# kei312/stereoanywhere

Measured on AMD Instinct MI355X. Metric: stereo pairs/sec @540x960 D=192 (1/2/4/8 GPU) + EPE vs reference, higher is better.
Workload: dtype f32 (F(4x4) Winograd-domain and direct-conv products as exact f16 hi/lo pair products on MFMA, fp32 accumulation; everything else fp32); 1 GPU; configs[1]: batch 4/GPU x 540x960 (padded 544x960), 22 GRU iters, published flags; global_batch=4, iters=22, parallelism=dp1 (independent pairs, metrics all_gather)

## Files before the change

### stereoanywhere_amd/csrc/conv_direct.hip

```cpp
#include "sa_common.h"

#pragma clang fp contract(fast)

namespace {

using sa::f32x4, sa::f32x2, sa::f16x2, sa::f16x4;

constexpr float DSP_SCALE = 4096.0f;
__device__ __forceinline__ f16x4 dsplit(const float x) {
  const f16x2 hh = __builtin_convertvector(f32x2{x, x}, f16x2);
  float l;
  asm("v_fma_mix_f32 %0, -%1, 1.0, %2 op_sel_hi:[1,0,0]" : "=v"(l) : "v"(__builtin_bit_cast(unsigned, hh)), "v"(x));
  const f16x2 ll = __builtin_convertvector(f32x2{l, l}, f16x2);
  return __builtin_shufflevector(hh, ll, 0, 1, 2, 3);
}

__device__ __forceinline__ float dunsplit(const float packed) {
  const f16x2 p = __builtin_bit_cast(f16x2, packed);
  return (float)p[0] + (float)p[1];
}

__device__ unsigned g_direct_redo_blocks;

constexpr int DOTH = 8, DOTW = 32, MT = 2;

template <int K, int S, int KC, int NTL, bool DS>
struct DCfg {
  static constexpr int PH = (DOTH - 1) * S + K, PW = (DOTW - 1) * S + K;
  static constexpr int PWP = PW;
  static constexpr int PL0 = PH * PWP, PR = S == 1 ? 16 : 17;
  static constexpr int PLANE = PL0 + ((PR - PL0 % 32) + 32) % 32;
  static constexpr int XN = KC * PLANE;
  static constexpr int NC = 16 * NTL;
  static constexpr int KK = K * K;
  static constexpr int WN = KC * KK * NC;
  static constexpr int DN = DS ? KC * NC : 0;
  static constexpr int NCP = NC + 16;
  static constexpr int WROWS = KC * KK + (DS ? KC : 0);
  static constexpr int XPT = (XN + 511) / 512, WPT = (WN + DN) / 4 / 512 + (((WN + DN) / 4) % 512 ? 1 : 0);
  static constexpr int KSTEPS = KC * KK / 4;
  static constexpr int NACC = NTL * (DS ? 2 : 1);
  static constexpr int SMEM = XN + WROWS * NCP + 4;
  static_assert(KC % 4 == 0, "a K-step of 4 must stay inside one tap");
  static_assert((WN + DN) % 4 == 0, "weights are staged as float4");
  static_assert(SMEM * 4 <= 160 * 1024, "LDS budget");
  static_assert(8 * 2 * NACC * 16 * 2 <= SMEM, "the stats reduction reuses the staging LDS");
};

struct DirArgs {
  const float *in;
  long in_bs;
  const float *skip, *cm, *cs;
  long skip_bs;
  int Cin, H, W, Ho, Wo;
  const float *wg, *wd;
  int Cout, co_blocks, tiles_w, tiles, nchunks;
  float *out, *out_ds;
  long out_bs, out_ds_bs;
  double *part, *part_ds;
};

__device__ __forceinline__ float close_value(float v, float m, float s, float k) {
#pragma clang fp contract(off)
  const float y = fmaxf((v - m) * s + 0.0f, 0.0f);
  return fmaxf(y + k, 0.0f);
}

template <int K, int S, int KC, int NTL, bool DS, bool SP = false, bool CL = false>
__global__ __launch_bounds__(512, DS ? 2 : 4) void conv_direct_kernel(const DirArgs a) {
  using C = DCfg<K, S, KC, NTL, DS>;
  constexpr int NC = C::NC, NCP = C::NCP, PLANE = C::PLANE, PWP = C::PWP;
  __shared__ __attribute__((aligned(16))) float sm[C::SMEM];
  __shared__ float ctab[CL ? 2 : 1][CL ? 2 * KC : 1];
  float *sx = sm, *sw = sm + C::XN, *sd = sw + KC * C::KK * NCP;
  constexpr int SPARE = C::SMEM - 4;
  const int tid = threadIdx.x, lane = tid & 63;
  const int wv = __builtin_amdgcn_readfirstlane(tid >> 6);
  const unsigned wid = sa::xcd_remap(blockIdx.x, gridDim.x);
  const int cb = wid % a.co_blocks;
  const int st = (wid / a.co_blocks) % a.tiles;
  const int n = wid / (a.co_blocks * a.tiles);
  const int oy0 = (st / a.tiles_w) * DOTH, ox0 = (st % a.tiles_w) * DOTW;
  const int iy0 = oy0 * S - K / 2, ix0 = ox0 * S - K / 2;
  const long hw = (long)a.H * a.W;
  const float *src = a.in + (long)n * a.in_bs;

  constexpr int OOB = 0x7ffffff0;
  const __amdgpu_buffer_rsrc_t xin = __builtin_amdgcn_make_buffer_rsrc(
      const_cast<float *>(src), (short)0, (int)((long)a.Cin * hw * 4), 0x00020000);
  int xoff[C::XPT], xl[C::XPT];
#pragma unroll
  for (int j = 0; j < C::XPT; ++j) {
    const int i = tid + 512 * j;
    const int ci = i / PLANE, rem = i % PLANE, r = rem / PWP, c = rem % PWP;
    const int y = iy0 + r, x = ix0 + c;
    const bool ok = i < C::XN && rem < C::PH * PWP && c < C::PW && y >= 0 && y < a.H && x >= 0 && x < a.W;
    xoff[j] = ok ? (int)((min(ci, a.Cin - 1) * hw + (long)y * a.W + x) * 4) : OOB;
    xl[j] = i < C::XN ? i : SPARE;
  }
  constexpr int WQ = (C::WN + C::DN) / 4;
  const __amdgpu_buffer_rsrc_t win = __builtin_amdgcn_make_buffer_rsrc(
      const_cast<float *>(a.wg) + (long)cb * a.nchunks * C::WN, (short)0, (int)((long)a.nchunks * C::WN * 4),
      0x00020000);
  const __amdgpu_buffer_rsrc_t din = __builtin_amdgcn_make_buffer_rsrc(
      const_cast<float *>(DS ? a.wd + (long)cb * a.nchunks * C::DN : a.wg), (short)0,
      (int)((long)a.nchunks * (DS ? C::DN : 0) * 4), 0x00020000);
  int woff[C::WPT], wl[C::WPT];
  bool wds[C::WPT];
#pragma unroll
  for (int j = 0; j < C::WPT; ++j) {
    const int i = tid + 512 * j;
    wds[j] = i >= C::WN / 4;
    woff[j] = i < WQ ? (wds[j] ? (i - C::WN / 4) * 16 : i * 16) : OOB;
    const int row = (4 * i) / NC, col = (4 * i) % NC;
    wl[j] = i < WQ ? row * NCP + col : SPARE;
  }
  const __amdgpu_buffer_rsrc_t kin = __builtin_amdgcn_make_buffer_rsrc(
      const_cast<float *>(CL ? a.skip + (long)n * a.skip_bs : src), (short)0, (int)((long)a.Cin * hw * 4), 0x00020000);
  float xr[C::XPT], kr[CL ? C::XPT : 1];
  float tv = 0.0f;
  f32x4 wr[C::WPT];
  auto fetch = [&](int chunk) __attribute__((always_inline)) {
    const int xs = chunk * KC * (int)hw * 4;
#pragma unroll
    for (int j = 0; j < C::XPT; ++j) xr[j] = __uint_as_float(__builtin_amdgcn_raw_buffer_load_b32(xin, xoff[j], xs, 0));
    if constexpr (CL) {
#pragma unroll
      for (int j = 0; j < C::XPT; ++j) kr[j] = __uint_as_float(__builtin_amdgcn_raw_buffer_load_b32(kin, xoff[j], xs, 0));
      if (tid < 2 * KC) {
        const int c = min(chunk * KC + tid % KC, a.Cin - 1);
        tv = (tid < KC ? a.cm : a.cs)[(long)n * a.Cin + c];
      }
    }
#pragma unroll
    for (int j = 0; j < C::WPT; ++j) {
      const auto v = wds[j] ? __builtin_amdgcn_raw_buffer_load_b128(din, woff[j], chunk * C::DN * 4, 0)
                            : __builtin_amdgcn_raw_buffer_load_b128(win, woff[j], chunk * C::WN * 4, 0);
      wr[j] = f32x4{__uint_as_float(v[0]), __uint_as_float(v[1]), __uint_as_float(v[2]), __uint_as_float(v[3])};
    }
  };
  auto put_tab = [&](int chunk) __attribute__((always_inline)) {
    if (CL && tid < 2 * KC) ctab[CL ? chunk & 1 : 0][tid] = tv;
  };
  auto commit = [&](int chunk) __attribute__((always_inline)) {
#pragma unroll
    for (int j = 0; j < C::XPT; ++j) {
      float v = xr[j];
      if constexpr (CL) {
        const int cl = min((tid + 512 * j) / PLANE, KC - 1);
        const float *tb = ctab[chunk & 1];
        v = xoff[j] == OOB ? 0.0f : close_value(v, tb[cl], tb[KC + cl], kr[j]);
      }
      sx[xl[j]] = v;
    }
#pragma unroll
    for (int j = 0; j < C::WPT; ++j) *reinterpret_cast<f32x4 *>(sw + wl[j]) = wr[j];
  };

  f32x4 acc[MT][C::NACC];
#pragma unroll
  for (int m = 0; m < MT; ++m)
#pragma unroll
    for (int t = 0; t < C::NACC; ++t) acc[m][t] = f32x4{0.f, 0.f, 0.f, 0.f};
  const int kq = lane >> 4, ml = lane & 15;
  int abase[MT];
#pragma unroll
  for (int m = 0; m < MT; ++m) abase[m] = kq * PLANE + (wv * S) * PWP + (m * 16 + ml) * S;
  const int bbase = kq * NCP + ml;

  fetch(0);
  if constexpr (CL) {
    put_tab(0);
    __syncthreads();
  }
  commit(0);
  __syncthreads();
#pragma unroll 1
  for (int chunk = 0; chunk < a.nchunks; ++chunk) {
    if (chunk + 1 < a.nchunks) fetch(chunk + 1);
#pragma unroll
    for (int s = 0; s < C::KSTEPS; ++s) {
      const int tap = (4 * s) / KC, ci0 = (4 * s) % KC;
      const int koff = ci0 * PLANE + (tap / K) * PWP + (tap % K);
      float av[MT];
#pragma unroll
      for (int m = 0; m < MT; ++m) av[m] = sx[abase[m] + koff];
      auto prod = [&](const float bv, f32x4 *ac) __attribute__((always_inline)) {
        if constexpr (SP) {
          const f16x4 b = __builtin_bit_cast(f16x4, f32x2{bv, bv});
#pragma unroll
          for (int m = 0; m < MT; ++m) ac[m * C::NACC] = __builtin_amdgcn_mfma_f32_16x16x16f16(dsplit(av[m]), b, ac[m * C::NACC], 0, 0, 0);
        } else {
#pragma unroll
          for (int m = 0; m < MT; ++m) ac[m * C::NACC] = __builtin_amdgcn_mfma_f32_16x16x4f32(av[m], bv, ac[m * C::NACC], 0, 0, 0);
        }
      };
#pragma unroll
      for (int t = 0; t < NTL; ++t) prod(sw[bbase + 4 * s * NCP + t * 16], &acc[0][t]);
      if (DS && tap == (K / 2) * K + K / 2) {
#pragma unroll
        for (int t = 0; t < NTL; ++t) prod(sd[bbase + ci0 * NCP + t * 16], &acc[0][NTL + t]);
      }
    }
    if (CL && chunk + 1 < a.nchunks) put_tab(chunk + 1);
    __syncthreads();
    if (chunk + 1 < a.nchunks) {
      commit(chunk + 1);
      __syncthreads();
    }
  }
  if constexpr (SP) {
    f32x4 sum = f32x4{0.f, 0.f, 0.f, 0.f};
#pragma unroll
    for (int m = 0; m < MT; ++m)
#pragma unroll
      for (int t = 0; t < C::NACC; ++t) sum += acc[m][t];
    const float tot = (sum.x + sum.y) + (sum.z + sum.w);
    if (__syncthreads_or(!__builtin_isfinite(tot))) {
      if (tid == 0) atomicAdd(&g_direct_redo_blocks, 1u);
#pragma unroll
      for (int m = 0; m < MT; ++m)
#pragma unroll
        for (int t = 0; t < C::NACC; ++t) acc[m][t] = f32x4{0.f, 0.f, 0.f, 0.f};
#pragma unroll 1
      for (int chunk = 0; chunk < a.nchunks; ++chunk) {
        fetch(chunk);
        if constexpr (CL) {
          put_tab(chunk);
          __syncthreads();
        }
        commit(chunk);
        __syncthreads();
#pragma unroll 1
        for (int s = 0; s < C::KSTEPS; ++s) {
          const int tap = (4 * s) / KC, ci0 = (4 * s) % KC;
          const int koff = ci0 * PLANE + (tap / K) * PWP + (tap % K);
#pragma unroll
          for (int t = 0; t < NTL; ++t) {
            const float w = dunsplit(sw[bbase + 4 * s * NCP + t * 16]);
#pragma unroll
            for (int m = 0; m < MT; ++m)
              acc[m][t] = __builtin_amdgcn_mfma_f32_16x16x4f32(sx[abase[m] + koff], w, acc[m][t], 0, 0, 0);
          }
          if (DS && tap == (K / 2) * K + K / 2) {
#pragma unroll
            for (int t = 0; t < NTL; ++t) {
              const float w = dunsplit(sd[bbase + ci0 * NCP + t * 16]);
#pragma unroll
              for (int m = 0; m < MT; ++m)
                acc[m][NTL + t] = __builtin_amdgcn_mfma_f32_16x16x4f32(sx[abase[m] + koff], w, acc[m][NTL + t], 0, 0, 0);
            }
          }
        }
        __syncthreads();
      }
    }
  }

  if constexpr (SP) {
#pragma unroll
    for (int m = 0; m < MT; ++m)
#pragma unroll
      for (int t = 0; t < C::NACC; ++t) acc[m][t] *= 1.0f / DSP_SCALE;
  }
  double *red = reinterpret_cast<double *>(sm);
  constexpr int RC = C::NACC * 16;
  const int oy = oy0 + wv;
  const bool stats = a.part != nullptr;
  const bool interior = oy0 + DOTH <= a.Ho && ox0 + DOTW <= a.Wo && (a.Wo & 3) == 0;
#pragma unroll
  for (int t = 0; t < C::NACC; ++t) {
    const bool ds = DS && t >= NTL;
    const int co = cb * NC + (ds ? t - NTL : t) * 16 + ml;
    float *dst = (ds ? a.out_ds + (long)n * a.out_ds_bs : a.out + (long)n * a.out_bs) + (long)co * a.Ho * a.Wo;
    double s1 = 0.0, s2 = 0.0;
    if (interior) {
#pragma unroll
      for (int m = 0; m < MT; ++m) {
        const int ox = ox0 + m * 16 + 4 * kq;
        *reinterpret_cast<float4 *>(dst + (long)oy * a.Wo + ox) =
            make_float4(acc[m][t][0], acc[m][t][1], acc[m][t][2], acc[m][t][3]);
#pragma unroll
        for (int r = 0; r < 4; ++r) {
          const double v = acc[m][t][r];
          s1 += v;
          s2 += v * v;
        }
      }
    } else {
#pragma unroll
      for (int m = 0; m < MT; ++m) {
        const int ox = ox0 + m * 16 + 4 * kq;
#pragma unroll
        for (int r = 0; r < 4; ++r) {
          if (oy < a.Ho && ox + r < a.Wo) {
            const float v = acc[m][t][r];
            dst[(long)oy * a.Wo + ox + r] = v;
            s1 += (double)v;
            s2 += (double)v * v;
          }
        }
      }
    }
    if (stats) {
      s1 += __shfl_xor(s1, 16);
      s2 += __shfl_xor(s2, 16);
      s1 += __shfl_xor(s1, 32);
      s2 += __shfl_xor(s2, 32);
      if (kq == 0) {
        red[(wv * 2 + 0) * RC + t * 16 + ml] = s1;
        red[(wv * 2 + 1) * RC + t * 16 + ml] = s2;
      }
    }
  }
  if (stats) {
    __syncthreads();
    for (int c = tid; c < RC; c += 512) {
      double s1 = 0.0, s2 = 0.0;
#pragma unroll
      for (int w = 0; w < 8; ++w) {
        s1 += red[(w * 2 + 0) * RC + c];
        s2 += red[(w * 2 + 1) * RC + c];
      }
      const bool ds = DS && c >= NC;
      double *pp = ds ? a.part_ds : a.part;
      if (pp) {
        const int co = cb * NC + (ds ? c - NC : c);
        pp += (((long)n * a.Cout + co) * a.tiles + st) * 2;
        pp[0] = s1;
        pp[1] = s2;
      }
    }
  }
}

__global__ void direct_weights_kernel(const float *__restrict__ w, int Cout, int Cin, int K, int KC, int NC,
                                      int nchunks, int ds, float *__restrict__ out) {
  const long total = (long)Cout * nchunks * KC * K * K;
  const long i = (long)blockIdx.x * blockDim.x + threadIdx.x;
  if (i >= total) return;
  const int n = (int)(i % NC);
  long r = i / NC;
  const int ci = (int)(r % KC);
  r /= KC;
  const int tap = (int)(r % (K * K));
  r /= K * K;
  const int chunk = (int)(r % nchunks);
  const int cblk = (int)(r / nchunks);
  const int co = cblk * NC + n, cin = chunk * KC + ci;
  (void)ds;
  out[i] = cin < Cin ? w[((long)co * Cin + cin) * K * K + tap] : 0.0f;
}

bool pick(int K, int S, int Cout, int &KC, int &NTL) {
  KC = K == 7 ? 4 : 8;
  if (K == 7 && S == 1 && Cout % 64 == 0) { NTL = 4; return true; }
  if ((K == 3 || K == 1) && S == 2 && Cout == 96) { NTL = 6; return true; }
  if ((K == 3 || K == 1) && S == 2 && Cout % 128 == 0) { NTL = 8; return true; }
  return false;
}

}

extern "C" int sa_conv_direct_weights(const float *weight, int Cout, int Cin, int K, int S, int with_ds,
                                      float *out, void *stream) {
  int KC = 0, NTL = 0;
  SA_REQUIRE(weight && out && Cout > 0 && Cin > 0, "sa_conv_direct_weights: bad arguments");
  SA_REQUIRE(pick(K, S, Cout, KC, NTL) && (K != 1 || with_ds), "sa_conv_direct_weights: no kernel for K=%d S=%d Cout=%d",
             K, S, Cout);
  const int NC = 16 * NTL, nchunks = (Cin + KC - 1) / KC;
  const long total = (long)Cout * nchunks * KC * K * K;
  hipStream_t s = sa::as_stream(stream);
  direct_weights_kernel<<<(unsigned)((total + 255) / 256), 256, 0, s>>>(weight, Cout, Cin, K, KC, NC, nchunks, 0,
                                                                       out);
  return sa::check_launch("sa_conv_direct_weights");
}

namespace {
__global__ void direct_split_kernel(const float *__restrict__ w, long n, unsigned *__restrict__ out) {
  const long i = (long)blockIdx.x * blockDim.x + threadIdx.x;
  if (i >= n) return;
  const double u = (double)w[i] * DSP_SCALE;
  const _Float16 hi = (_Float16)(float)u;
  const _Float16 lo = (_Float16)(float)(u - (double)hi);
  out[i] = (unsigned)__builtin_bit_cast(unsigned short, hi) | ((unsigned)__builtin_bit_cast(unsigned short, lo) << 16);
}

}

extern "C" int sa_conv_direct_weights_split(const float *arranged, long n, void *out, void *stream) {
  SA_REQUIRE(arranged && out && n > 0, "sa_conv_direct_weights_split: bad arguments");
  hipStream_t s = sa::as_stream(stream);
  direct_split_kernel<<<(unsigned)((n + 255) / 256), 256, 0, s>>>(arranged, n, static_cast<unsigned *>(out));
  return sa::check_launch("sa_conv_direct_weights_split");
}

long sa_direct_redo_blocks_internal(int reset) {
  return sa::read_redo_counter(g_direct_redo_blocks, reset, false);
}

extern "C" long sa_conv_direct_weights_size(int Cout, int Cin, int K, int S, int with_ds) {
  int KC = 0, NTL = 0;
  if (!pick(K, S, Cout, KC, NTL) || (K == 1 && !with_ds)) return -1;
  return (long)Cout * ((Cin + KC - 1) / KC) * KC * K * K;
}

extern "C" long sa_conv_direct_stat_parts(int Ho, int Wo) {
  return (long)((Wo + DOTW - 1) / DOTW) * ((Ho + DOTH - 1) / DOTH);
}

template <bool SP>
static int conv_direct_launch(const float *in, long in_bs, int N, int Cin, int H, int W, int K, int S,
                              const float *wg, const float *wd, int Cout, float *out, long out_bs, float *out_ds,
                              long out_ds_bs, double *part, double *part_ds, void *stream,
                              const float *skip = nullptr, long skip_bs = 0, const float *cm = nullptr,
                              const float *cs = nullptr) {
  int KC = 0, NTL = 0;
  const bool ds = wd != nullptr, cl = skip != nullptr;
  SA_REQUIRE(in && wg && out && N > 0 && Cin > 0 && H > 0 && W > 0, "sa_conv_direct: bad arguments");
  SA_REQUIRE(!ds || out_ds, "sa_conv_direct: downsample weights without an output");
  SA_REQUIRE(K != 1 && pick(K, S, Cout, KC, NTL) && ds == (S == 2),
             "sa_conv_direct: no kernel for K=%d S=%d Cout=%d ds=%d", K, S, Cout, (int)ds);
  SA_REQUIRE((long)Cin * H * W < (1L << 31), "sa_conv_direct: image too large");
  SA_REQUIRE(Cin % KC == 0 || Cin <= KC, "sa_conv_direct: Cin must be a multiple of %d (or at most %d)", KC, KC);
  SA_REQUIRE(!cl || (cm && cs && K == 3 && Cin % KC == 0),
             "sa_conv_direct_close: needs mean / rstd, a 3x3 stride-2 conv and Cin %% %d == 0", KC);
  const int p = K / 2;
  const int Ho = (H + 2 * p - K) / S + 1, Wo = (W + 2 * p - K) / S + 1;
  const int tiles_w = (Wo + DOTW - 1) / DOTW, tiles = tiles_w * ((Ho + DOTH - 1) / DOTH);
  const int co_blocks = Cout / (16 * NTL);
  const DirArgs a{in, in_bs, skip, cm, cs, skip_bs, Cin, H, W, Ho, Wo, wg, wd, Cout, co_blocks, tiles_w, tiles,
                  (Cin + KC - 1) / KC, out, out_ds, out_bs, out_ds_bs, part, part_ds};
  const long nblk = (long)N * tiles * co_blocks;
  SA_REQUIRE(nblk < (1L << 31), "sa_conv_direct: grid too large");
  hipStream_t s = sa::as_stream(stream);
  sa::TimingScope ts(SA_K_CONV_DIRECT, s);
  if (K == 7) {
    conv_direct_kernel<7, 1, 4, 4, false, SP><<<(unsigned)nblk, 512, 0, s>>>(a);
  } else if (NTL == 6) {
    if (cl) conv_direct_kernel<3, 2, 8, 6, true, SP, true><<<(unsigned)nblk, 512, 0, s>>>(a);
    else conv_direct_kernel<3, 2, 8, 6, true, SP><<<(unsigned)nblk, 512, 0, s>>>(a);
  } else {
    SA_REQUIRE(!cl, "sa_conv_direct_close: no close form for Cout = %d", Cout);
    conv_direct_kernel<3, 2, 8, 8, true, SP><<<(unsigned)nblk, 512, 0, s>>>(a);
  }
  return sa::check_launch("sa_conv_direct");
}

extern "C" int sa_conv_direct(const float *in, long in_bs, int N, int Cin, int H, int W, int K, int S,
                              const float *wg, const float *wd, int Cout, float *out, long out_bs, float *out_ds,
                              long out_ds_bs, double *part, double *part_ds, void *stream) {
  return conv_direct_launch<false>(in, in_bs, N, Cin, H, W, K, S, wg, wd, Cout, out, out_bs, out_ds, out_ds_bs, part,
                                   part_ds, stream);
}

extern "C" int sa_conv_direct_split(const float *in, long in_bs, int N, int Cin, int H, int W, int K, int S,
                                    const void *wg, const void *wd, int Cout, float *out, long out_bs, float *out_ds,
                                    long out_ds_bs, double *part, double *part_ds, void *stream) {
  return conv_direct_launch<true>(in, in_bs, N, Cin, H, W, K, S, static_cast<const float *>(wg),
                                  static_cast<const float *>(wd), Cout, out, out_bs, out_ds, out_ds_bs, part, part_ds,
                                  stream);
}

extern "C" int sa_conv_direct_close_supported(int K, int S, int Cout) {
  int KC = 0, NTL = 0;
  return K == 3 && S == 2 && pick(K, S, Cout, KC, NTL) && NTL == 6 ? 1 : 0;
}

extern "C" int sa_conv_direct_close(const float *c2, long c2_bs, const float *skip, long skip_bs, const float *mean,
                                    const float *rstd, int N, int Cin, int H, int W, int K, int S, const void *wg,
                                    const void *wd, int split, int Cout, float *out, long out_bs, float *out_ds,
                                    long out_ds_bs, double *part, double *part_ds, void *stream) {
  SA_REQUIRE(skip, "sa_conv_direct_close: null skip");
  if (split)
    return conv_direct_launch<true>(c2, c2_bs, N, Cin, H, W, K, S, static_cast<const float *>(wg),
                                    static_cast<const float *>(wd), Cout, out, out_bs, out_ds, out_ds_bs, part, part_ds,
                                    stream, skip, skip_bs, mean, rstd);
  return conv_direct_launch<false>(c2, c2_bs, N, Cin, H, W, K, S, static_cast<const float *>(wg),
                                   static_cast<const float *>(wd), Cout, out, out_bs, out_ds, out_ds_bs, part, part_ds,
                                   stream, skip, skip_bs, mean, rstd);
}
```

Measured before the change: 71.48 pairs/s.

## Add K=32 f16 hi/lo MFMA direct-conv kernel for split-precision path

Adds a new direct-convolution kernel for the split-precision (SP) path. It stages input patches and weights in LDS as separate f16 hi/lo planes, then computes each tap row with three 16x16x32 f16 MFMAs (hi*hi, hi*lo, lo*hi), replacing per-element 16x16x16 MFMAs that split operands at runtime. This cuts the MFMA instruction count and the in-loop conversion work. In exchange it adds more complex LDS layout and staging code, and a redo path with a new range check (overflow or small-magnitude inputs) that falls back to fp32 MFMA. The epilogue is factored into a shared helper.

New measurement: 71.82 pairs/s (median of 6 runs). No clear change (+0.5%).

```diff
diff --git a/stereoanywhere_amd/csrc/conv_direct.hip b/stereoanywhere_amd/csrc/conv_direct.hip
--- a/stereoanywhere_amd/csrc/conv_direct.hip
+++ b/stereoanywhere_amd/csrc/conv_direct.hip
@@ -7,18 +7,6 @@
 using sa::f32x4, sa::f32x2, sa::f16x2, sa::f16x4;
 
 constexpr float DSP_SCALE = 4096.0f;
-__device__ __forceinline__ f16x4 dsplit(const float x) {
-  const f16x2 hh = __builtin_convertvector(f32x2{x, x}, f16x2);
-  float l;
-  asm("v_fma_mix_f32 %0, -%1, 1.0, %2 op_sel_hi:[1,0,0]" : "=v"(l) : "v"(__builtin_bit_cast(unsigned, hh)), "v"(x));
-  const f16x2 ll = __builtin_convertvector(f32x2{l, l}, f16x2);
-  return __builtin_shufflevector(hh, ll, 0, 1, 2, 3);
-}
-
-__device__ __forceinline__ float dunsplit(const float packed) {
-  const f16x2 p = __builtin_bit_cast(f16x2, packed);
-  return (float)p[0] + (float)p[1];
-}
 
 __device__ unsigned g_direct_redo_blocks;
 
@@ -66,7 +54,83 @@
   return fmaxf(y + k, 0.0f);
 }
 
-template <int K, int S, int KC, int NTL, bool DS, bool SP = false, bool CL = false>
+template <int NTL, bool DS>
+__device__ __forceinline__ void direct_epilogue(const DirArgs &a, f32x4 (&acc)[MT][NTL * (DS ? 2 : 1)], double *red,
+                                                const int tid, const int wv, const int n, const int cb, const int st,
+                                                const int oy0, const int ox0) {
+  constexpr int NC = 16 * NTL, NACC = NTL * (DS ? 2 : 1);
+  const int lane = tid & 63, kq = lane >> 4, ml = lane & 15;
+  constexpr int RC = NACC * 16;
+  const int oy = oy0 + wv;
+  const bool stats = a.part != nullptr;
+  const bool interior = oy0 + DOTH <= a.Ho && ox0 + DOTW <= a.Wo && (a.Wo & 3) == 0;
+#pragma unroll
+  for (int t = 0; t < NACC; ++t) {
+    const bool ds = DS && t >= NTL;
+    const int co = cb * NC + (ds ? t - NTL : t) * 16 + ml;
+    float *dst = (ds ? a.out_ds + (long)n * a.out_ds_bs : a.out + (long)n * a.out_bs) + (long)co * a.Ho * a.Wo;
+    double s1 = 0.0, s2 = 0.0;
+    if (interior) {
+#pragma unroll
+      for (int m = 0; m < MT; ++m) {
+        const int ox = ox0 + m * 16 + 4 * kq;
+        *reinterpret_cast<float4 *>(dst + (long)oy * a.Wo + ox) =
+            make_float4(acc[m][t][0], acc[m][t][1], acc[m][t][2], acc[m][t][3]);
+#pragma unroll
+        for (int r = 0; r < 4; ++r) {
+          const double v = acc[m][t][r];
+          s1 += v;
+          s2 += v * v;
+        }
+      }
+    } else {
+#pragma unroll
+      for (int m = 0; m < MT; ++m) {
+        const int ox = ox0 + m * 16 + 4 * kq;
+#pragma unroll
+        for (int r = 0; r < 4; ++r) {
+          if (oy < a.Ho && ox + r < a.Wo) {
+            const float v = acc[m][t][r];
+            dst[(long)oy * a.Wo + ox + r] = v;
+            s1 += (double)v;
+            s2 += (double)v * v;
+          }
+        }
+      }
+    }
+    if (stats) {
+      s1 += __shfl_xor(s1, 16);
+      s2 += __shfl_xor(s2, 16);
+      s1 += __shfl_xor(s1, 32);
+      s2 += __shfl_xor(s2, 32);
+      if (kq == 0) {
+        red[(wv * 2 + 0) * RC + t * 16 + ml] = s1;
+        red[(wv * 2 + 1) * RC + t * 16 + ml] = s2;
+      }
+    }
+  }
+  if (stats) {
+    __syncthreads();
+    for (int c = tid; c < RC; c += 512) {
+      double s1 = 0.0, s2 = 0.0;
+#pragma unroll
+      for (int w = 0; w < 8; ++w) {
+        s1 += red[(w * 2 + 0) * RC + c];
+        s2 += red[(w * 2 + 1) * RC + c];
+      }
+      const bool ds = DS && c >= NC;
+      double *pp = ds ? a.part_ds : a.part;
+      if (pp) {
+        const int co = cb * NC + (ds ? c - NC : c);
+        pp += (((long)n * a.Cout + co) * a.tiles + st) * 2;
+        pp[0] = s1;
+        pp[1] = s2;
+      }
+    }
+  }
+}
+
+template <int K, int S, int KC, int NTL, bool DS, bool CL = false>
 __global__ __launch_bounds__(512, DS ? 2 : 4) void conv_direct_kernel(const DirArgs a) {
   using C = DCfg<K, S, KC, NTL, DS>;
   constexpr int NC = C::NC, NCP = C::NCP, PLANE = C::PLANE, PWP = C::PWP;
@@ -186,14 +250,8 @@
 #pragma unroll
       for (int m = 0; m < MT; ++m) av[m] = sx[abase[m] + koff];
       auto prod = [&](const float bv, f32x4 *ac) __attribute__((always_inline)) {
-        if constexpr (SP) {
-          const f16x4 b = __builtin_bit_cast(f16x4, f32x2{bv, bv});
-#pragma unroll
-          for (int m = 0; m < MT; ++m) ac[m * C::NACC] = __builtin_amdgcn_mfma_f32_16x16x16f16(dsplit(av[m]), b, ac[m * C::NACC], 0, 0, 0);
-        } else {
-#pragma unroll
-          for (int m = 0; m < MT; ++m) ac[m * C::NACC] = __builtin_amdgcn_mfma_f32_16x16x4f32(av[m], bv, ac[m * C::NACC], 0, 0, 0);
-        }
+#pragma unroll
+        for (int m = 0; m < MT; ++m) ac[m * C::NACC] = __builtin_amdgcn_mfma_f32_16x16x4f32(av[m], bv, ac[m * C::NACC], 0, 0, 0);
       };
 #pragma unroll
       for (int t = 0; t < NTL; ++t) prod(sw[bbase + 4 * s * NCP + t * 16], &acc[0][t]);
@@ -209,129 +267,305 @@
       __syncthreads();
     }
   }
-  if constexpr (SP) {
-    f32x4 sum = f32x4{0.f, 0.f, 0.f, 0.f};
+  direct_epilogue<NTL, DS>(a, acc, reinterpret_cast<double *>(sm), tid, wv, n, cb, st, oy0, ox0);
+}
+
+template <int K, int S, int NTL, bool DS>
+struct K32Cfg {
+  static constexpr int KC = K == 7 ? 4 : 8;
+  static constexpr int TPG = 8 / KC;
+  static constexpr int TC = 4 * TPG;
+  static constexpr int GR = (K + TPG - 1) / TPG;
+  static constexpr int PH = (DOTH - 1) * S + K, PWR = (DOTW - 1) * S + K, PW = (DOTW - 1) * S + TC;
+  static constexpr int SLOTB = 2 * KC;
+  static constexpr int IMGB = PW * SLOTB, ROWB = 2 * IMGB;
+  static constexpr int X0 = (IMGB + 16 + 15) / 16 * 16;
+  static constexpr int XB = PH * ROWB, W0 = X0 + XB;
+  static constexpr int RH = 8 / KC, RPT = PH / RH;
+  static constexpr int CX = PW > 64 ? PW - 64 : 0, EXTRA = KC * PH * CX, EPT = EXTRA ? 1 : 0;
+  static_assert(RPT * RH == PH && EXTRA <= 512, "every patch value has one staging slot");
+  static constexpr int NC = 16 * NTL, NACC = NTL * (DS ? 2 : 1);
+  static constexpr int WN = KC * K * K * NC, DN = DS ? KC * NC : 0;
+  static constexpr int WROWS = 4 * (K + (DS ? 1 : 0));
+  static constexpr int WIMG = WROWS * NC * 16;
+  static constexpr int UNITS = K * GR * NC + (DS ? NC : 0), WPT = (UNITS + 511) / 512;
+  static constexpr int SMEMB = W0 + 2 * WIMG;
+  static_assert(TC >= K && (S == 1 || PW % 2 == 0), "a tap row fits one step");
+  static_assert(XB % 16 == 0 && SMEMB <= 160 * 1024, "LDS budget");
+  static_assert(8 * 2 * NACC * 16 * 8 <= SMEMB, "the stats reduction reuses the staging LDS");
+};
+
+using sa::f16x8;
+using u32x4 = __attribute__((ext_vector_type(4))) unsigned;
+
+template <int K, int S, int NTL, bool DS, bool CL = false>
+__global__ __launch_bounds__(512, DS ? 2 : 4) void conv_direct_k32_kernel(const DirArgs a) {
+  using C = K32Cfg<K, S, NTL, DS>;
+  constexpr int KC = C::KC, NC = C::NC, PW = C::PW, ROWB = C::ROWB, IMGB = C::IMGB, SLOTB = C::SLOTB;
+  constexpr int X0 = C::X0, W0 = C::W0, WIMG = C::WIMG;
+  __shared__ __attribute__((aligned(16))) unsigned char smb[C::SMEMB];
+  __shared__ float ctab[CL ? 2 : 1][CL ? 2 * KC : 1];
+  const int tid = threadIdx.x, lane = tid & 63;
+  const int wv = __builtin_amdgcn_readfirstlane(tid >> 6);
+  const unsigned wid = sa::xcd_remap(blockIdx.x, gridDim.x);
+  const int cb = wid % a.co_blocks;
+  const int st = (wid / a.co_blocks) % a.tiles;
+  const int n = wid / (a.co_blocks * a.tiles);
+  const int oy0 = (st / a.tiles_w) * DOTH, ox0 = (st % a.tiles_w) * DOTW;
+  const int iy0 = oy0 * S - K / 2, ix0 = ox0 * S - K / 2;
+  const long hw = (long)a.H * a.W;
+  const float *src = a.in + (long)n * a.in_bs;
+
+  constexpr int OOB = 0x7ffffff0;
+  const __amdgpu_buffer_rsrc_t xin = __builtin_amdgcn_make_buffer_rsrc(
+      const_cast<float *>(src), (short)0, (int)((long)a.Cin * hw * 4), 0x00020000);
+  auto slot_of = [](const int c) { return S == 2 ? (c & 1) * (PW / 2) + (c >> 1) : c; };
+  const int sci = wv % KC, srow0 = (wv / KC) * C::RPT;
+  const bool cok = lane < C::PWR && ix0 + lane >= 0 && ix0 + lane < a.W;
+  const int xoff = cok ? (int)((min(sci, a.Cin - 1) * hw + ix0 + lane) * 4) : OOB;
+  const int xl = X0 + srow0 * ROWB + slot_of(lane) * SLOTB + sci * 2;
+  auto row_ok = [&](const int k) { return iy0 + srow0 + k >= 0 && iy0 + srow0 + k < a.H; };
+  int eoff = OOB, el = 0, ecl = 0;
+  if constexpr (C::EPT) {
+    const int eci = tid / (C::PH * C::CX), rem = tid % (C::PH * C::CX), r = rem / C::CX, c = 64 + rem % C::CX;
+    const int y = iy0 + r, x = ix0 + c;
+    const bool ok = tid < C::EXTRA && c < C::PWR && y >= 0 && y < a.H && x >= 0 && x < a.W;
+    eoff = ok ? (int)((min(eci, a.Cin - 1) * hw + (long)y * a.W + x) * 4) : OOB;
+    el = tid < C::EXTRA ? X0 + r * ROWB + slot_of(c) * SLOTB + eci * 2 : 0;
+    ecl = min(eci, KC - 1);
+  }
+  const unsigned *wgb = reinterpret_cast<const unsigned *>(a.wg) + (long)cb * a.nchunks * C::WN;
+  const unsigned *wdb = DS ? reinterpret_cast<const unsigned *>(a.wd) + (long)cb * a.nchunks * C::DN : wgb;
+  unsigned wu[C::WPT];
+  static_assert(C::WN + C::DN < 65536 && (W0 + WIMG) / 16 < 65535, "weight units are packed in one register");
+  bool wds[C::WPT], wpad[C::WPT];
+#pragma unroll
+  for (int j = 0; j < C::WPT; ++j) {
+    const int u = tid + 512 * j;
+    const bool valid = u < C::UNITS;
+    wds[j] = DS && valid && u >= K * C::GR * NC;
+    const int v = !valid ? 0 : wds[j] ? u - K * C::GR * NC : u;
+    const int nn = v % NC, sg = v / NC, s = sg / C::GR, g = sg % C::GR;
+    const unsigned wo = wds[j] ? nn : (s * K + g * C::TPG) * KC * NC + nn;
+    wpad[j] = C::TPG == 2 && g * 2 + 1 >= K;
+    wu[j] = wo | (valid ? (unsigned)(W0 / 16 + (wds[j] ? 4 * K + 1 : s * 4 + g) * NC + nn) << 16 : 0xffff0000u);
+  }
+  const __amdgpu_buffer_rsrc_t kin = __builtin_amdgcn_make_buffer_rsrc(
+      const_cast<float *>(CL ? a.skip + (long)n * a.skip_bs : src), (short)0, (int)((long)a.Cin * hw * 4), 0x00020000);
+  constexpr int XPT = C::RPT + C::EPT;
+  float xr[XPT], kr[CL ? XPT : 1];
+  float tv = 0.0f;
+  unsigned wr[C::WPT][8];
+  auto fetch_x = [&](int chunk) __attribute__((always_inline)) {
+    const int xs = chunk * KC * (int)hw * 4;
+#pragma unroll
+    for (int k = 0; k < C::RPT; ++k) {
+      const int so = xs + min(max(iy0 + srow0 + k, 0), a.H - 1) * a.W * 4;
+      xr[k] = __uint_as_float(__builtin_amdgcn_raw_buffer_load_b32(xin, xoff, so, 0));
+      if constexpr (CL) kr[k] = __uint_as_float(__builtin_amdgcn_raw_buffer_load_b32(kin, xoff, so, 0));
+    }
+    if constexpr (C::EPT) {
+      xr[C::RPT] = __uint_as_float(__builtin_amdgcn_raw_buffer_load_b32(xin, eoff, xs, 0));
+      if constexpr (CL) kr[C::RPT] = __uint_as_float(__builtin_amdgcn_raw_buffer_load_b32(kin, eoff, xs, 0));
+    }
+    if constexpr (CL) {
+      if (tid < 2 * KC) {
+        const int c = min(chunk * KC + tid % KC, a.Cin - 1);
+        tv = (tid < KC ? a.cm : a.cs)[(long)n * a.Cin + c];
+      }
+    }
+  };
+  auto fetch_w = [&](int chunk, const int j0, const int j1) __attribute__((always_inline)) {
+#pragma unroll
+    for (int j = j0; j < j1; ++j) {
+      const unsigned *p = wds[j] ? wdb : wgb;
+      const int o = (int)(wu[j] & 0xffffu) + chunk * (wds[j] ? C::DN : C::WN);
+      const int o2 = o + (wpad[j] ? 0 : 4 * NC);
+#pragma unroll
+      for (int q = 0; q < 8; ++q) wr[j][q] = q < 4 ? p[o + q * NC] : p[o2 + (q - 4) * NC];
+    }
+  };
+  auto put_tab = [&](int chunk) __attribute__((always_inline)) {
+    if (CL && tid < 2 * KC) ctab[CL ? chunk & 1 : 0][tid] = tv;
+  };
+  float amax = 0.0f;
+  auto commit_x = [&](int chunk, const bool raw) __attribute__((always_inline)) {
+    auto put = [&](float v, const float k, const bool ok, const int cl, const int la) __attribute__((always_inline)) {
+      if constexpr (CL) {
+        const float *tb = ctab[chunk & 1];
+        v = ok ? close_value(v, tb[cl], tb[KC + cl], k) : 0.0f;
+      } else {
+        v = ok ? v : 0.0f;
+      }
+      unsigned short h, l;
+      if (raw) {
+        h = (unsigned short)(__float_as_uint(v) & 0xffffu);
+        l = (unsigned short)(__float_as_uint(v) >> 16);
+      } else {
+        amax = fmaxf(amax, fabsf(v));
+        const _Float16 hf = (_Float16)v;
+        const _Float16 lf = (_Float16)(v - (float)hf);
+        h = __builtin_bit_cast(unsigned short, hf);
+        l = __builtin_bit_cast(unsigned short, lf);
+      }
+      *reinterpret_cast<unsigned short *>(smb + la) = h;
+      *reinterpret_cast<unsigned short *>(smb + la + IMGB) = l;
+    };
+    if (PW >= 64 || lane < PW) {
+#pragma unroll
+      for (int k = 0; k < C::RPT; ++k) put(xr[k], kr[CL ? k : 0], cok && row_ok(k), sci, xl + k * ROWB);
+    }
+    if constexpr (C::EPT) put(xr[C::RPT], kr[CL ? C::RPT : 0], eoff != OOB, ecl, el);
+  };
+  auto commit_w = [&](const int j0, const int j1) __attribute__((always_inline)) {
+#pragma unroll
+    for (int j = j0; j < j1; ++j) {
+      u32x4 h, l;
+#pragma unroll
+      for (int q = 0; q < 4; ++q) {
+        h[q] = (wr[j][2 * q] & 0xffffu) | (wr[j][2 * q + 1] << 16);
+        l[q] = (wr[j][2 * q] >> 16) | (wr[j][2 * q + 1] & 0xffff0000u);
+        if (C::TPG == 2 && q >= 2 && wpad[j]) h[q] = l[q] = 0u;
+      }
+      if (wu[j] < 0xffff0000u) {
+        *reinterpret_cast<u32x4 *>(smb + (wu[j] >> 16) * 16) = h;
+        *reinterpret_cast<u32x4 *>(smb + (wu[j] >> 16) * 16 + WIMG) = l;
+      }
+    }
+  };
+
+  const int kq = lane >> 4, ml = lane & 15;
+  const int aslot = S == 2 ? (kq & 1) * (PW / 2) + ml + (kq >> 1) : ml + kq * C::TPG;
+  const int abase = X0 + (wv * S) * ROWB + aslot * SLOTB;
+  const int bbase = W0 + (kq * NC + ml) * 16;
+  auto read_a = [&](const int off) __attribute__((always_inline)) -> u32x4 {
+    if constexpr (SLOTB == 16) {
+      return *reinterpret_cast<const u32x4 *>(smb + off);
+    } else {
+      const auto p = *reinterpret_cast<const uint2 *>(smb + off), q = *reinterpret_cast<const uint2 *>(smb + off + 8);
+      return u32x4{p.x, p.y, q.x, q.y};
+    }
+  };
+
+  constexpr int H2 = K == 7 ? C::WPT / 2 : C::WPT;
+  auto stage = [&](int chunk, const bool raw) __attribute__((always_inline)) {
+    fetch_x(chunk);
+    fetch_w(chunk, 0, H2);
+    if constexpr (CL) {
+      put_tab(chunk);
+      __syncthreads();
+    }
+    commit_x(chunk, raw);
+    commit_w(0, H2);
+    if constexpr (H2 < C::WPT) {
+      fetch_w(chunk, H2, C::WPT);
+      commit_w(H2, C::WPT);
+    }
+    __syncthreads();
+  };
+  if constexpr (C::UNITS < C::WROWS * NC) {
+    for (int i = tid * 16; i < 2 * WIMG; i += 512 * 16) *reinterpret_cast<u32x4 *>(smb + W0 + i) = u32x4{0u, 0u, 0u, 0u};
+    __syncthreads();
+  }
+  stage(0, false);
+  constexpr int AS = K / 2;
+  f32x4 acc[MT][C::NACC];
+#pragma unroll
+  for (int m = 0; m < MT; ++m)
+#pragma unroll
+    for (int t = 0; t < C::NACC; ++t) acc[m][t] = f32x4{0.f, 0.f, 0.f, 0.f};
+#pragma unroll 1
+  for (int chunk = 0; chunk < a.nchunks; ++chunk) {
+    if (K != 7 && chunk + 1 < a.nchunks) {
+      fetch_x(chunk + 1);
+      fetch_w(chunk + 1, 0, C::WPT);
+    }
+    auto step = [&](const int aoff, const int boff, f32x4 *ac) __attribute__((always_inline)) {
+      f16x8 ah[MT], al[MT];
+#pragma unroll
+      for (int m = 0; m < MT; ++m) {
+        ah[m] = __builtin_bit_cast(f16x8, read_a(aoff + m * 16 * SLOTB));
+        al[m] = __builtin_bit_cast(f16x8, read_a(aoff + m * 16 * SLOTB + IMGB));
+      }
+#pragma unroll
+      for (int t = 0; t < NTL; ++t) {
+        const f16x8 bh = *reinterpret_cast<const f16x8 *>(smb + boff + t * 256);
+        const f16x8 bl = *reinterpret_cast<const f16x8 *>(smb + boff + t * 256 + WIMG);
+#pragma unroll
+        for (int m = 0; m < MT; ++m) ac[m * C::NACC + t] = __builtin_amdgcn_mfma_f32_16x16x32_f16(ah[m], bh, ac[m * C::NACC + t], 0, 0, 0);
+#pragma unroll
+        for (int m = 0; m < MT; ++m) ac[m * C::NACC + t] = __builtin_amdgcn_mfma_f32_16x16x32_f16(ah[m], bl, ac[m * C::NACC + t], 0, 0, 0);
+#pragma unroll
+        for (int m = 0; m < MT; ++m) ac[m * C::NACC + t] = __builtin_amdgcn_mfma_f32_16x16x32_f16(al[m], bh, ac[m * C::NACC + t], 0, 0, 0);
+      }
+    };
+    if constexpr (K == 7) {
+#pragma unroll 1
+      for (int s = 0; s < K; ++s) step(abase + s * ROWB, bbase + s * 4 * NC * 16, &acc[0][0]);
+    } else {
+#pragma unroll
+      for (int s = 0; s < K; ++s) step(abase + s * ROWB, bbase + s * 4 * NC * 16, &acc[0][0]);
+    }
+    if constexpr (DS) step(abase + AS * ROWB, bbase + K * 4 * NC * 16, &acc[0][NTL]);
+    if (CL && chunk + 1 < a.nchunks) put_tab(chunk + 1);
+    __syncthreads();
+    if (chunk + 1 < a.nchunks) {
+      if constexpr (K == 7) {
+        stage(chunk + 1, false);
+      } else {
+        commit_x(chunk + 1, false);
+        commit_w(0, C::WPT);
+        __syncthreads();
+      }
+    }
+  }
+  const int over = __syncthreads_or(!(amax < 65504.0f));
+  const int large = __syncthreads_or(amax >= 0.03125f);
+  const int nonzero = __syncthreads_or(amax > 0.0f);
+  if (over || (!large && nonzero)) {
+    if (tid == 0) atomicAdd(&g_direct_redo_blocks, 1u);
 #pragma unroll
     for (int m = 0; m < MT; ++m)
 #pragma unroll
-      for (int t = 0; t < C::NACC; ++t) sum += acc[m][t];
-    const float tot = (sum.x + sum.y) + (sum.z + sum.w);
-    if (__syncthreads_or(!__builtin_isfinite(tot))) {
-      if (tid == 0) atomicAdd(&g_direct_redo_blocks, 1u);
-#pragma unroll
-      for (int m = 0; m < MT; ++m)
-#pragma unroll
-        for (int t = 0; t < C::NACC; ++t) acc[m][t] = f32x4{0.f, 0.f, 0.f, 0.f};
+      for (int t = 0; t < C::NACC; ++t) acc[m][t] = f32x4{0.f, 0.f, 0.f, 0.f};
+    auto redo_step = [&](const int aoff, const int boff, f32x4 *ac) __attribute__((always_inline)) {
+      float av[MT][8];
+#pragma unroll
+      for (int m = 0; m < MT; ++m) {
+        const u32x4 lo = read_a(aoff + m * 16 * SLOTB), hi = read_a(aoff + m * 16 * SLOTB + IMGB);
+#pragma unroll
+        for (int q = 0; q < 4; ++q) {
+          av[m][2 * q] = __uint_as_float((lo[q] & 0xffffu) | (hi[q] << 16));
+          av[m][2 * q + 1] = __uint_as_float((lo[q] >> 16) | (hi[q] & 0xffff0000u));
+        }
+      }
+#pragma unroll
+      for (int t = 0; t < NTL; ++t) {
+        const f16x8 bh = *reinterpret_cast<const f16x8 *>(smb + boff + t * 256);
+        const f16x8 bl = *reinterpret_cast<const f16x8 *>(smb + boff + t * 256 + WIMG);
+#pragma unroll
+        for (int q = 0; q < 8; ++q) {
+          const float w = (float)bh[q] + (float)bl[q];
+#pragma unroll
+          for (int m = 0; m < MT; ++m)
+            ac[m * C::NACC + t] = __builtin_amdgcn_mfma_f32_16x16x4f32(av[m][q], w, ac[m * C::NACC + t], 0, 0, 0);
+        }
+      }
+    };
 #pragma unroll 1
-      for (int chunk = 0; chunk < a.nchunks; ++chunk) {
-        fetch(chunk);
-        if constexpr (CL) {
-          put_tab(chunk);
-          __syncthreads();
-        }
-        commit(chunk);
-        __syncthreads();
+    for (int chunk = 0; chunk < a.nchunks; ++chunk) {
+      stage(chunk, true);
 #pragma unroll 1
-        for (int s = 0; s < C::KSTEPS; ++s) {
-          const int tap = (4 * s) / KC, ci0 = (4 * s) % KC;
-          const int koff = ci0 * PLANE + (tap / K) * PWP + (tap % K);
-#pragma unroll
-          for (int t = 0; t < NTL; ++t) {
-            const float w = dunsplit(sw[bbase + 4 * s * NCP + t * 16]);
-#pragma unroll
-            for (int m = 0; m < MT; ++m)
-              acc[m][t] = __builtin_amdgcn_mfma_f32_16x16x4f32(sx[abase[m] + koff], w, acc[m][t], 0, 0, 0);
-          }
-          if (DS && tap == (K / 2) * K + K / 2) {
-#pragma unroll
-            for (int t = 0; t < NTL; ++t) {
-              const float w = dunsplit(sd[bbase + ci0 * NCP + t * 16]);
-#pragma unroll
-              for (int m = 0; m < MT; ++m)
-                acc[m][NTL + t] = __builtin_amdgcn_mfma_f32_16x16x4f32(sx[abase[m] + koff], w, acc[m][NTL + t], 0, 0, 0);
-            }
-          }
-        }
-        __syncthreads();
-      }
-    }
-  }
-
-  if constexpr (SP) {
-#pragma unroll
-    for (int m = 0; m < MT; ++m)
-#pragma unroll
-      for (int t = 0; t < C::NACC; ++t) acc[m][t] *= 1.0f / DSP_SCALE;
-  }
-  double *red = reinterpret_cast<double *>(sm);
-  constexpr int RC = C::NACC * 16;
-  const int oy = oy0 + wv;
-  const bool stats = a.part != nullptr;
-  const bool interior = oy0 + DOTH <= a.Ho && ox0 + DOTW <= a.Wo && (a.Wo & 3) == 0;
-#pragma unroll
-  for (int t = 0; t < C::NACC; ++t) {
-    const bool ds = DS && t >= NTL;
-    const int co = cb * NC + (ds ? t - NTL : t) * 16 + ml;
-    float *dst = (ds ? a.out_ds + (long)n * a.out_ds_bs : a.out + (long)n * a.out_bs) + (long)co * a.Ho * a.Wo;
-    double s1 = 0.0, s2 = 0.0;
-    if (interior) {
-#pragma unroll
-      for (int m = 0; m < MT; ++m) {
-        const int ox = ox0 + m * 16 + 4 * kq;
-        *reinterpret_cast<float4 *>(dst + (long)oy * a.Wo + ox) =
-            make_float4(acc[m][t][0], acc[m][t][1], acc[m][t][2], acc[m][t][3]);
-#pragma unroll
-        for (int r = 0; r < 4; ++r) {
-          const double v = acc[m][t][r];
-          s1 += v;
-          s2 += v * v;
-        }
-      }
-    } else {
-#pragma unroll
-      for (int m = 0; m < MT; ++m) {
-        const int ox = ox0 + m * 16 + 4 * kq;
-#pragma unroll
-        for (int r = 0; r < 4; ++r) {
-          if (oy < a.Ho && ox + r < a.Wo) {
-            const float v = acc[m][t][r];
-            dst[(long)oy * a.Wo + ox + r] = v;
-            s1 += (double)v;
-            s2 += (double)v * v;
-          }
-        }
-      }
-    }
-    if (stats) {
-      s1 += __shfl_xor(s1, 16);
-      s2 += __shfl_xor(s2, 16);
-      s1 += __shfl_xor(s1, 32);
-      s2 += __shfl_xor(s2, 32);
-      if (kq == 0) {
-        red[(wv * 2 + 0) * RC + t * 16 + ml] = s1;
-        red[(wv * 2 + 1) * RC + t * 16 + ml] = s2;
-      }
-    }
-  }
-  if (stats) {
-    __syncthreads();
-    for (int c = tid; c < RC; c += 512) {
-      double s1 = 0.0, s2 = 0.0;
-#pragma unroll
-      for (int w = 0; w < 8; ++w) {
-        s1 += red[(w * 2 + 0) * RC + c];
-        s2 += red[(w * 2 + 1) * RC + c];
-      }
-      const bool ds = DS && c >= NC;
-      double *pp = ds ? a.part_ds : a.part;
-      if (pp) {
-        const int co = cb * NC + (ds ? c - NC : c);
-        pp += (((long)n * a.Cout + co) * a.tiles + st) * 2;
-        pp[0] = s1;
-        pp[1] = s2;
-      }
-    }
-  }
+      for (int s = 0; s < K; ++s) redo_step(abase + s * ROWB, bbase + s * 4 * NC * 16, &acc[0][0]);
+      if constexpr (DS) redo_step(abase + AS * ROWB, bbase + K * 4 * NC * 16, &acc[0][NTL]);
+      __syncthreads();
+    }
+  }
+#pragma unroll
+  for (int m = 0; m < MT; ++m)
+#pragma unroll
+    for (int t = 0; t < C::NACC; ++t) acc[m][t] *= 1.0f / DSP_SCALE;
+  direct_epilogue<NTL, DS>(a, acc, reinterpret_cast<double *>(smb), tid, wv, n, cb, st, oy0, ox0);
 }
 
 __global__ void direct_weights_kernel(const float *__restrict__ w, int Cout, int Cin, int K, int KC, int NC,
@@ -435,14 +669,24 @@
   SA_REQUIRE(nblk < (1L << 31), "sa_conv_direct: grid too large");
   hipStream_t s = sa::as_stream(stream);
   sa::TimingScope ts(SA_K_CONV_DIRECT, s);
-  if (K == 7) {
-    conv_direct_kernel<7, 1, 4, 4, false, SP><<<(unsigned)nblk, 512, 0, s>>>(a);
+  if constexpr (SP) {
+    if (K == 7) {
+      conv_direct_k32_kernel<7, 1, 4, false><<<(unsigned)nblk, 512, 0, s>>>(a);
+    } else if (NTL == 6) {
+      if (cl) conv_direct_k32_kernel<3, 2, 6, true, true><<<(unsigned)nblk, 512, 0, s>>>(a);
+      else conv_direct_k32_kernel<3, 2, 6, true><<<(unsigned)nblk, 512, 0, s>>>(a);
+    } else {
+      SA_REQUIRE(!cl, "sa_conv_direct_close: no close form for Cout = %d", Cout);
+      conv_direct_k32_kernel<3, 2, 8, true><<<(unsigned)nblk, 512, 0, s>>>(a);
+    }
+  } else if (K == 7) {
+    conv_direct_kernel<7, 1, 4, 4, false><<<(unsigned)nblk, 512, 0, s>>>(a);
   } else if (NTL == 6) {
-    if (cl) conv_direct_kernel<3, 2, 8, 6, true, SP, true><<<(unsigned)nblk, 512, 0, s>>>(a);
-    else conv_direct_kernel<3, 2, 8, 6, true, SP><<<(unsigned)nblk, 512, 0, s>>>(a);
+    if (cl) conv_direct_kernel<3, 2, 8, 6, true, true><<<(unsigned)nblk, 512, 0, s>>>(a);
+    else conv_direct_kernel<3, 2, 8, 6, true><<<(unsigned)nblk, 512, 0, s>>>(a);
   } else {
     SA_REQUIRE(!cl, "sa_conv_direct_close: no close form for Cout = %d", Cout);
-    conv_direct_kernel<3, 2, 8, 8, true, SP><<<(unsigned)nblk, 512, 0, s>>>(a);
+    conv_direct_kernel<3, 2, 8, 8, true><<<(unsigned)nblk, 512, 0, s>>>(a);
   }
   return sa::check_launch("sa_conv_direct");
 }
```
